# sauloal/pykmer

Measured on AMD Instinct MI355X. Metric: bp/s k-mer counted (k=15, 1 GPU), higher is better.
Workload: dtype u8

## Files before the change

pykmer_amd/csrc/kmer_part.hip:

```cpp
#include <cstddef>
#include "part_common.h"

namespace pk {

__global__ __launch_bounds__(1024) void k_sample2(const uint32_t *__restrict__ in, const uint32_t *__restrict__ bucket_base,
                                                  const uint32_t *__restrict__ bucket_end, PartPlan pl, uint32_t stride2,
                                                  uint32_t *__restrict__ tally, uint32_t *__restrict__ sampled_n,
                                                  const uint32_t *__restrict__ flags) {
    __shared__ uint32_t h[512];
    __shared__ uint32_t n_seen;
    if (flags[0]) return;
    const uint32_t b = blockIdx.x, lo = bucket_base[b], hi = bucket_end[b];
    if (threadIdx.x < 512) h[threadIdx.x] = 0;
    if (threadIdx.x == 0) n_seen = 0;
    __syncthreads();
    const uint32_t n_grp = (hi - lo + 255u) / 256u, n_sgrp = (n_grp + stride2 - 1u) / stride2;
    const uint32_t mask = pl.B2 - 1u, shift = pl.fb_bits, w = threadIdx.x >> 6, lane = threadIdx.x & 63u;
    uint32_t mine = 0;
    for (uint32_t s0 = 0; s0 < n_sgrp; s0 += 8u * 16u) {
        uint4 v[8];
        uint32_t n_ok[8];
#pragma unroll
        for (int u = 0; u < 8; u++) {
            const uint32_t sg = s0 + (uint32_t)u * 16u + w;
            const uint64_t i = (uint64_t)lo + (uint64_t)sg * stride2 * 256u + lane * 4u;
            n_ok[u] = (sg < n_sgrp && i < hi) ? (uint32_t)min((uint64_t)4, (uint64_t)hi - i) : 0u;
            v[u] = n_ok[u] ? *reinterpret_cast<const uint4 *>(in + i) : make_uint4(0, 0, 0, 0);
        }
#pragma unroll
        for (int u = 0; u < 8; u++) {
            const uint32_t r4[4] = {v[u].x, v[u].y, v[u].z, v[u].w};
#pragma unroll
            for (uint32_t e = 0; e < 4; e++)
                if (e < n_ok[u]) { atomicAdd(&h[(r4[e] >> shift) & mask], 1u); mine++; }
        }
    }
    for (int d = 32; d; d >>= 1) mine += __shfl_down(mine, d, 64);
    if ((threadIdx.x & 63) == 0 && mine) atomicAdd(&n_seen, mine);
    __syncthreads();
    if (threadIdx.x < pl.B2) tally[(uint64_t)b * pl.B2 + threadIdx.x] = h[threadIdx.x];
    if (threadIdx.x == 0) sampled_n[b] = n_seen;
}
__global__ __launch_bounds__(1024) void k_rooms2(const uint32_t *__restrict__ tally, const uint32_t *__restrict__ sampled_n,
                                                 const uint32_t *__restrict__ bucket_base, const uint32_t *__restrict__ bucket_end, PartPlan pl,
                                                 uint32_t stride2, uint32_t n_final, uint32_t *__restrict__ final_start,
                                                 uint32_t *__restrict__ cap2_end, uint32_t *__restrict__ block_tot, const uint32_t *__restrict__ flags) {
    __shared__ uint32_t wsum[16];
    if (flags[0]) return;
    const uint32_t i = blockIdx.x * 1024u + threadIdx.x;
    uint32_t room = 0;
    if (i < n_final) {
        const uint32_t b = i >> pl.b2, hcount = tally[i];
        if (stride2 == 1u) room = hcount;
        else {
            const uint32_t seen = sampled_n[b], n_b = bucket_end[b] - bucket_base[b];
            const unsigned long long est = seen ? (unsigned long long)((double)hcount * ((double)n_b / (double)seen)) + 1ull : 0ull;
            room = (uint32_t)(est + est / 4 + 4096u);
        }
        room = (room + 7u) & ~7u;
    }
    uint32_t inc = room;
    const int lane = threadIdx.x & 63, w = threadIdx.x >> 6;
#pragma unroll
    for (int d = 1; d < 64; d <<= 1) { const uint32_t o = __shfl_up(inc, d, 64); if (lane >= d) inc += o; }
    if (lane == 63) wsum[w] = inc;
    __syncthreads();
    uint32_t pre = 0, total = 0;
    for (int j = 0; j < 16; j++) { if (j < w) pre += wsum[j]; total += wsum[j]; }
    if (i < n_final) { final_start[i] = pre + inc - room; cap2_end[i] = room; }
    if (threadIdx.x == 0) block_tot[blockIdx.x] = total;
}
__global__ __launch_bounds__(1024) void k_bases2(uint32_t n_blocks, uint32_t n_final, PartPlan pl, uint32_t *__restrict__ block_tot,
                                                 uint32_t *__restrict__ final_start, uint32_t *__restrict__ flags) {
    __shared__ uint32_t wsum[16];
    if (flags[0]) return;
    const uint32_t v = threadIdx.x < n_blocks ? block_tot[threadIdx.x] : 0u;
    uint32_t inc = v;
    const int lane = threadIdx.x & 63, w = threadIdx.x >> 6;
#pragma unroll
    for (int d = 1; d < 64; d <<= 1) { const uint32_t o = __shfl_up(inc, d, 64); if (lane >= d) inc += o; }
    if (lane == 63) wsum[w] = inc;
    __syncthreads();
    uint32_t pre = 0, total = 0;
    for (int j = 0; j < 16; j++) { if (j < w) pre += wsum[j]; total += wsum[j]; }
    if (threadIdx.x < n_blocks) block_tot[threadIdx.x] = pre + inc - v;
    __shared__ unsigned long long total64;
    if (threadIdx.x == 0) total64 = 0ull;
    __syncthreads();
    unsigned long long mine = v;
    for (int d = 32; d; d >>= 1) mine += __shfl_down(mine, d, 64);
    if (lane == 0 && mine) atomicAdd(&total64, mine);
    __syncthreads();
    if (threadIdx.x == 0) {
        final_start[n_final] = total;
        if (total64 > pl.capacity2) flags[0] = 1u;
    }
}
__global__ __launch_bounds__(1024) void k_starts2(uint32_t n_final, const uint32_t *__restrict__ block_base, uint32_t *__restrict__ final_start,
                                                  uint32_t *__restrict__ cursor2, uint32_t *__restrict__ cap2_end, const uint32_t *__restrict__ flags) {
    if (flags[0]) return;
    const uint32_t i = blockIdx.x * 1024u + threadIdx.x;
    if (i >= n_final) return;
    const uint32_t a = block_base[blockIdx.x] + final_start[i];
    final_start[i] = a; cursor2[i] = a; cap2_end[i] = a + cap2_end[i];
}

template <int NT, int PER, bool REC24 = false>
__global__ __launch_bounds__(NT, 4) void k_scatter2(const uint32_t *__restrict__ in, const uint32_t *__restrict__ wg2_start,
                                                   const uint32_t *__restrict__ bucket_base, const uint32_t *__restrict__ bucket_end, PartPlan pl,
                                                   void *__restrict__ out, uint32_t *__restrict__ cursor, const uint32_t *__restrict__ cap_end,
                                                   uint32_t dump, uint32_t *__restrict__ flags) {
    extern __shared__ __attribute__((aligned(16))) uint8_t smem[];
    ScatterLds &L = *reinterpret_cast<ScatterLds *>(smem);
    if (flags[0]) return;
    const uint32_t B = pl.B2, shift = pl.fb_bits;
    const uint32_t low_mask = (1u << shift) - 1u;
    for (uint32_t i = threadIdx.x; i < 512; i += NT) { L.hist[i] = 0; L.run[i] = 0; }
    __syncthreads();
    typedef uint32_t Quad __attribute__((ext_vector_type(4)));
    typedef uint32_t Pair __attribute__((ext_vector_type(2)));
    const uint16_t *in_lo = reinterpret_cast<const uint16_t *>(in);
    const uint8_t *in_hi = reinterpret_cast<const uint8_t *>(in) + level1_hi_plane_offset(pl.capacity1);
    auto item = [&](uint32_t b, uint32_t lo, uint32_t hi) {
        auto fetch = [&](uint32_t win, Quad (&v)[PER / 4]) {
            const uint32_t v_hi = min(hi, win + (uint32_t)TILE);
#pragma unroll
            for (int j = 0; j < PER / 4; j++) {
                const uint32_t i = win + (threadIdx.x + j * NT) * 4u;
                v[j] = Quad{0u, 0u, 0u, 0u};
                if (i < v_hi) {
                    if (REC24) {
                        const Pair l = *reinterpret_cast<const Pair *>(in_lo + i);
                        v[j] = Quad{l.x, l.y, *reinterpret_cast<const uint32_t *>(in_hi + i), 0u};
                    } else v[j] = *reinterpret_cast<const Quad *>(in + i);
                }
            }
        };
        Quad nxt[PER / 4];
        auto settle = [&]() {
            __builtin_amdgcn_s_waitcnt(0x0F70);
#pragma unroll
            for (int j = 0; j < PER / 4; j++) asm volatile("" : "+v"(nxt[j]));
        };
        fetch(lo & ~3u, nxt);
        settle();
        for (uint32_t win = lo & ~3u; win < hi; win += TILE) {
            const uint32_t v_lo = max(lo, win), v_hi = min(hi, win + (uint32_t)TILE);
            const uint32_t n_tile = v_hi - v_lo;
            uint32_t r[PER];
#pragma unroll
            for (int j = 0; j < PER / 4; j++) {
                if (REC24) {
                    r[j * 4] = __builtin_amdgcn_perm(nxt[j].z, nxt[j].x, 0x0c040100u);
                    r[j * 4 + 1] = __builtin_amdgcn_perm(nxt[j].z, nxt[j].x, 0x0c050302u);
                    r[j * 4 + 2] = __builtin_amdgcn_perm(nxt[j].z, nxt[j].y, 0x0c060100u);
                    r[j * 4 + 3] = __builtin_amdgcn_perm(nxt[j].z, nxt[j].y, 0x0c070302u);
                } else { r[j * 4] = nxt[j].x; r[j * 4 + 1] = nxt[j].y; r[j * 4 + 2] = nxt[j].z; r[j * 4 + 3] = nxt[j].w; }
            }
            const bool full = v_lo == win && n_tile == (uint32_t)TILE;
            uint32_t okm = 0;
            if (!full) {
#pragma unroll
                for (int j = 0; j < PER / 4; j++) {
                    const uint32_t i = win + (threadIdx.x + j * NT) * 4u;
#pragma unroll
                    for (int e = 0; e < 4; e++) okm |= (i + e >= v_lo && i + e < v_hi) ? (1u << (j * 4 + e)) : 0u;
                }
            }
            if (win + TILE < hi) fetch(win + TILE, nxt);
            uint32_t *cl = cursor + (uint64_t)b * B;
            const uint32_t *ce = cap_end + (uint64_t)b * B;
            if (full) scatter_tile<uint32_t, false, NT, PER, 512, true, 8, REC24>(L, r, 0u, n_tile, shift, B, low_mask, true, out, settle, cl, ce, dump, flags);
            else scatter_tile<uint32_t, false, NT, PER, 512, false, 8, REC24>(L, r, okm, n_tile, shift, B, low_mask, true, out, settle, cl, ce, dump, flags);
        }
    };
    const uint32_t *pos = wg2_start;
    const uint32_t per = pl.B1 >> 3;
    const uint32_t o_lo = (blockIdx.x & 7u) * per, o_hi = o_lo + per, first = blockIdx.x >> 3, step = gridDim.x >> 3;
    const uint32_t w_end = pos[o_hi];
    for (uint32_t w = pos[o_lo] + first; w < w_end; w += step) {
        uint32_t a = o_lo, z = o_hi;
        while (z - a > 1) { const uint32_t m = (a + z) >> 1; if (pos[m] <= w) a = m; else z = m; }
        const uint32_t b = (a % per) * 8u + a / per;
        const uint64_t s = (uint64_t)bucket_base[b] + (uint64_t)(w - pos[a]) * pl.R2;
        const uint64_t e = min(s + pl.R2, (uint64_t)bucket_end[b]);
        item(b, (uint32_t)s, (uint32_t)e);
    }
}

constexpr uint32_t K6_PIECE = 65024;
constexpr int K6_BYTES_LDS = 65536 + 1024 + 128;

__device__ __forceinline__ int wave_sum_i32(int v) {
    v += __builtin_amdgcn_update_dpp(0, v, 0x128, 0xf, 0xf, false);
    v += __builtin_amdgcn_update_dpp(0, v, 0x124, 0xf, 0xf, false);
    v += __builtin_amdgcn_update_dpp(0, v, 0x122, 0xf, 0xf, false);
    v += __builtin_amdgcn_update_dpp(0, v, 0x121, 0xf, 0xf, false);
    return __builtin_amdgcn_readlane(v, 0) + __builtin_amdgcn_readlane(v, 16) + __builtin_amdgcn_readlane(v, 32) +
           __builtin_amdgcn_readlane(v, 48);
}

typedef unsigned short U16x2 __attribute__((ext_vector_type(2)));
__device__ __forceinline__ uint32_t clamp255_pair(uint32_t x) {
    const U16x2 lim = {255, 255};
    return __builtin_bit_cast(uint32_t, __builtin_elementwise_min(__builtin_bit_cast(U16x2, x), lim));
}
__device__ __forceinline__ uint32_t pack_low_bytes(uint32_t x0, uint32_t x1) {
    return __builtin_amdgcn_perm(x1, x0, 0x06040200u);
}

struct SliceTally {
    int d1 = 0, d2 = 0;
    __device__ __forceinline__ void add_dword(int *dh, uint32_t x, int sign) {
        uint32_t p0 = x & 0x01010101u, p1 = (x >> 1) & 0x01010101u;
        uint32_t rest = p0 & p1;
        const uint32_t high = x & 0xfcfcfcfcu;
        if (high) {
            const uint32_t big = (((high & 0x7f7f7f7fu) + 0x7f7f7f7fu) | high) & 0x80808080u;
            const uint32_t keep = ~(big >> 7);
            p0 &= keep; p1 &= keep;
            rest = (p0 & p1) | (big >> 7);
        }
        const int n1 = (int)__builtin_popcount(p0 & ~p1), n2 = (int)__builtin_popcount(p1 & ~p0);
        d1 += sign * n1; d2 += sign * n2;
        while (rest) {
            const int bit = __ffs(rest) - 1;
            atomicAdd(&dh[(x >> bit) & 0xffu], sign);
            rest &= rest - 1u;
        }
    }
};

template <int T, bool LEAN, bool NOREC = false>
__device__ __forceinline__ void bucket_count_body(const uint16_t *__restrict__ recs, const uint32_t *__restrict__ final_start,
                                                  const uint32_t *__restrict__ final_end, uint32_t fb_bits, uint32_t split_bits,
                                                  uint8_t *__restrict__ table8, uint32_t fresh, unsigned long long *__restrict__ hist_rep, uint8_t *smem,
                                                  int *dh, uint32_t wg) {
    uint32_t *cnt = reinterpret_cast<uint32_t *>(smem);
    const uint32_t fb = wg >> split_bits, part = wg & ((1u << split_bits) - 1u);
    const uint32_t start = final_start[fb], end = final_end ? final_end[fb] : final_start[fb + 1];
    const uint32_t part_bits = fb_bits - split_bits;
    const uint32_t n_addr = 1u << part_bits;
    uint8_t *slice = table8 + ((uint64_t)fb << fb_bits) + (uint64_t)part * n_addr;
    if (start == end) {
        if (fresh) {
            if (n_addr >= 16) for (uint32_t g = threadIdx.x; g < n_addr / 16; g += T) reinterpret_cast<uint4 *>(slice)[g] = make_uint4(0, 0, 0, 0);
            else for (uint32_t a = threadIdx.x; a < n_addr; a += T) slice[a] = 0;
        }
        return;
    }
    const uint32_t base = start & ~7u;
    const uint32_t i_first = base + threadIdx.x * 8;
    uint4 v_first = make_uint4(0, 0, 0, 0);
    if (i_first < min(base + K6_PIECE, end)) v_first = *reinterpret_cast<const uint4 *>(recs + i_first);
    const bool by_rec = NOREC ? false : (((end - start) >> split_bits) < n_addr / 4 || n_addr < 16);
    SliceTally tally;
    for (uint32_t i = threadIdx.x; i < 256; i += T) dh[i] = 0;
    if (fresh) {
        if (n_addr >= 8) for (uint32_t g = threadIdx.x; g < n_addr / 8; g += T) reinterpret_cast<uint4 *>(cnt)[g] = make_uint4(0, 0, 0, 0);
        else for (uint32_t a = threadIdx.x; a < max(n_addr / 2, 1u); a += T) cnt[a] = 0u;
    } else if (n_addr >= 16) {
        if (!by_rec) __syncthreads();
        for (uint32_t g = threadIdx.x; g < n_addr / 16; g += T) {
            uint4 v = reinterpret_cast<const uint4 *>(slice)[g];
            uint32_t w[4] = {v.x, v.y, v.z, v.w};
            if (!by_rec) {
#pragma unroll
                for (int q = 0; q < 4; q++) tally.add_dword(dh, w[q], -1);
            }
#pragma unroll
            for (int q = 0; q < 8; q++)
                cnt[g * 8 + q] = __builtin_amdgcn_perm(0u, w[q >> 1], (q & 1) ? 0x0c030c02u : 0x0c010c00u);
        }
    } else {
        for (uint32_t a = threadIdx.x; a < n_addr / 2; a += T) cnt[a] = slice[2 * a] | ((uint32_t)slice[2 * a + 1] << 16);
    }
    __syncthreads();
    auto bump = [&](uint32_t a, uint32_t n) {
        const uint32_t sh = 16u * (a & 1u);
        if (!by_rec) { atomicAdd(&cnt[a >> 1], n << sh); return; }
        int &d1 = tally.d1, &d2 = tally.d2;
        const uint32_t c = (atomicAdd(&cnt[a >> 1], n << sh) >> sh) & 0xffffu;
        const uint32_t oc = c > 255u ? 255u : c, nc = c + n > 255u ? 255u : c + n;
        if (oc == nc) return;
        if (nc == 1u) d1++;
        else if (nc == 2u && oc == 1u) { d2++; d1--; }
        else {
            atomicAdd(&dh[nc], 1);
            if (oc) atomicAdd(&dh[oc], -1);
        }
    };
    auto count8 = [&](const uint4 &v, uint32_t i) {
        const uint32_t w[4] = {v.x, v.y, v.z, v.w};
        if (LEAN && !by_rec) {
            const bool interior = i >= start && i + 8u <= end;
            uint8_t *cb = reinterpret_cast<uint8_t *>(cnt);
#pragma unroll
            for (int q = 0; q < 8; q++) {
                const uint32_t x = w[q >> 1];
                const uint32_t off = (q & 1) ? ((x >> 15) & 0x1fffcu) : ((x << 1) & 0x1fffcu);
                const uint32_t low = (q & 1) ? ((x >> 16) & 1u) : (x & 1u);
                uint32_t val = low * 0xffffu + 1u;
                if (!interior) val = (i + q >= start && i + q < end) ? val : 0u;
                __hip_atomic_fetch_add(reinterpret_cast<uint32_t *>(cb + off), val, __ATOMIC_RELAXED, __HIP_MEMORY_SCOPE_WORKGROUP);
            }
            return;
        }
        uint32_t pa = 0, pn = 0;
#pragma unroll
        for (int q = 0; q < 8; q++) {
            const uint32_t idx = i + q;
            const uint32_t full = (w[q >> 1] >> (16 * (q & 1))) & 0xffffu;
            const bool in = idx >= start && idx < end && (full >> part_bits) == part;
            const uint32_t a = full & (n_addr - 1u);
            if (in && pn && a == pa) pn++;
            else {
                if (pn) bump(pa, pn);
                pa = a; pn = in ? 1u : 0u;
            }
        }
        if (pn) bump(pa, pn);
    };
    auto count8_sparse = [&](const uint4 &v, uint32_t i) {
        const uint32_t w[4] = {v.x, v.y, v.z, v.w};
        uint32_t old[8];
        bool in[8];
// ... 163 lines not shown
        return;
    }
    for (uint32_t g = threadIdx.x; g < N_ADDR / 16; g += T) slice[g] = img[g];
    d1 = wave_sum_i32(d1); d2 = wave_sum_i32(d2);
    if ((threadIdx.x & 63) == 0) {
        if (d1) atomicAdd(&dh[1], d1);
        if (d2) atomicAdd(&dh[2], d2);
    }
    __syncthreads();
    for (uint32_t i = threadIdx.x; i < 256; i += T) {
        const int x = dh[i];
        if (x) atomicAdd(&hist_rep[(uint64_t)(blockIdx.x % HIST_REPLICAS) * 256 + i], (unsigned long long)(long long)x);
    }
}

__device__ __forceinline__ void hist_reduce(unsigned long long *__restrict__ hist_rep, unsigned long long *__restrict__ hist) {
    if (threadIdx.x >= 256) return;
    unsigned long long acc = 0;
    for (uint32_t r = 0; r < HIST_REPLICAS; r++) {
        acc += hist_rep[(uint64_t)r * 256 + threadIdx.x];
        hist_rep[(uint64_t)r * 256 + threadIdx.x] = 0ull;
    }
    if (acc) atomicAdd(&hist[threadIdx.x], acc);
}

constexpr uint32_t AS_SLOTS = 4096, AS_WGS = 64;

__device__ __forceinline__ void table_sat_add(uint8_t *table8, uint64_t addr, uint32_t cnt, int *dh) {
    unsigned int *word = reinterpret_cast<unsigned int *>(table8 + (addr & ~3ull));
    const uint32_t sh = (uint32_t)(addr & 3ull) * 8u;
    unsigned int old = *word;
    while (true) {
        uint32_t b = (old >> sh) & 0xffu;
        uint32_t nb = b + cnt > 255u ? 255u : b + cnt;
        if (nb == b) return;
        unsigned int want = (old & ~(0xffu << sh)) | (nb << sh);
        unsigned int prev = atomicCAS(word, old, want);
        if (prev == old) {
            atomicAdd(&dh[nb], 1);
            if (b) atomicAdd(&dh[b], -1);
            return;
        }
        old = prev;
    }
}

__global__ __launch_bounds__(WG) void k_apply_side(const unsigned long long *__restrict__ side, const unsigned long long *__restrict__ side_n,
                                                   uint64_t side_cap, uint8_t *__restrict__ table8, unsigned long long *__restrict__ hist,
                                                   unsigned long long *__restrict__ hist_rep, const uint32_t *__restrict__ flags) {
    __shared__ unsigned long long key[AS_SLOTS];
    if (flags[0]) return;
    static_assert(WG >= 256, "one thread per histogram bin");
    if (blockIdx.x == 0) hist_reduce(hist_rep, hist);
    __shared__ uint32_t val[AS_SLOTS];
    __shared__ int dh[256];
    unsigned long long n = *side_n;
    if (n > side_cap) n = side_cap;
    const unsigned long long per = (n + gridDim.x - 1) / gridDim.x;
    const unsigned long long lo = per * blockIdx.x, hi = lo + per < n ? lo + per : n;
    if (lo >= hi) return;
    for (uint32_t i = threadIdx.x; i < AS_SLOTS; i += WG) { key[i] = 0ull; val[i] = 0u; }
    dh[threadIdx.x & 255u] = 0;
    __syncthreads();
    for (unsigned long long i = lo + threadIdx.x; i < hi; i += WG) {
        const unsigned long long e = side[i];
        const uint64_t addr = e >> SIDE_CNT_BITS;
        const uint32_t cnt = (uint32_t)(e & ((1ull << SIDE_CNT_BITS) - 1ull));
        const unsigned long long kk = addr + 1ull;
        uint32_t h = (uint32_t)((addr * 0x9E3779B97F4A7C15ull) >> 40) & (AS_SLOTS - 1u);
        bool done = false;
        for (uint32_t t = 0; t < 32 && !done; t++) {
            unsigned long long old = atomicCAS(&key[h], 0ull, kk);
            if (old == 0ull || old == kk) {
                uint32_t before = atomicAdd(&val[h], cnt);
                if (before + cnt < before) atomicExch(&val[h], 0xffffffffu);
                done = true;
            }
            h = (h + 1u) & (AS_SLOTS - 1u);
        }
        if (!done) table_sat_add(table8, addr, cnt > 255u ? 255u : cnt, dh);
    }
    __syncthreads();
    for (uint32_t i = threadIdx.x; i < AS_SLOTS; i += WG)
        if (key[i] != 0ull) table_sat_add(table8, key[i] - 1ull, val[i] > 255u ? 255u : val[i], dh);
    __syncthreads();
    if (threadIdx.x < 256 && dh[threadIdx.x]) atomicAdd(&hist[threadIdx.x], (unsigned long long)(long long)dh[threadIdx.x]);
}

PartPlan make_part_plan(uint32_t k, uint64_t n_bytes, uint32_t slice_bits, uint32_t slice_index) {
    PartPlan pl;
    pl.k = k;
    pl.slice_bits = slice_bits;
    pl.slice_index = slice_index;
    pl.addr_bits = 2 * k - slice_bits;
    pl.fb_bits = pl.addr_bits < 16 ? pl.addr_bits : 16;
    if (k <= 15 && pl.addr_bits >= 24 && n_bytes >= (((uint64_t)1 << pl.addr_bits) >> 3)) pl.fb_bits = 15;
    const uint32_t bucket_bits = pl.addr_bits - pl.fb_bits;
    const uint32_t one_level_max = k <= 15 ? 7u : 9u;
    pl.b1 = bucket_bits <= one_level_max ? bucket_bits : (bucket_bits + 1) / 2;
    if (pl.b1 > one_level_max) pl.b1 = one_level_max;
    pl.b2 = bucket_bits - pl.b1;
    pl.B1 = 1u << pl.b1;
    pl.B2 = 1u << pl.b2;
    pl.n_chunks = (uint32_t)((n_bytes + CHUNK - 1) / CHUNK);
    pl.n_wg0 = pl.n_chunks < 1024u ? pl.n_chunks : 1024u;
    if (pl.n_wg0 == 0) pl.n_wg0 = 1;
    pl.G = (pl.n_chunks + pl.n_wg0 - 1) / pl.n_wg0;
    if (pl.G == 0) pl.G = 1;
    const uint32_t wg1 = 4096u;
    pl.n_wg1 = pl.n_chunks < wg1 ? pl.n_chunks : wg1;
    if (pl.n_wg1 == 0) pl.n_wg1 = 1;
    pl.G1 = (pl.n_chunks + pl.n_wg1 - 1) / pl.n_wg1;
    if (pl.G1 == 0) pl.G1 = 1;
    pl.R2 = 4u * TILE;
    pl.sample_stride = pl.n_chunks >= 1024u ? 16u : 1u;
    const uint64_t nfb = (uint64_t)pl.B1 * pl.B2;
    pl.n_tally = (pl.b2 && nfb <= 32768 && pl.addr_bits <= 30) ? (uint32_t)nfb : pl.B1;
    pl.sample2 = (pl.b2 && pl.n_tally == pl.B1 && nfb <= 262144 && pl.B1 >= 8u) ? 1u : 0u;
    const uint64_t est1 = (uint64_t)pl.n_chunks * TILE + pl.B1, est2 = (uint64_t)pl.n_chunks * TILE + nfb;
    pl.capacity1 = est1 + est1 / 8 + (uint64_t)pl.B1 * 4100;
    pl.capacity2 = pl.sample2 ? est2 + est2 / 4 + nfb * 4104 : est2 + est2 / 8 + nfb * 2056;
    return pl;
}

size_t part_workspace_bytes(const PartPlan &pl, uint64_t n_bytes, PartWorkspace *lay) {
    auto up = [](size_t x) { return (x + 255) & ~(size_t)255; };
    const uint64_t nfb = (uint64_t)pl.B1 * pl.B2;
    size_t o = 0;
    lay->codes = o; o += up((size_t)pl.n_chunks * SLOT_CODE_WORDS * 4);
    lay->restarts = o; o += up((size_t)pl.n_chunks * SLOT_RST_WORDS * 4);
    lay->n_bases = o; o += up((size_t)pl.n_chunks * 4);
    lay->tally_rows = o; o += up((size_t)COUNT_WGS * pl.n_tally * 4);
    lay->tally_tot = o; o += up(pl.sample2 ? (size_t)nfb * 4 + (size_t)(pl.B1 + 1024) * 4 : (size_t)pl.n_tally * 4);
    lay->bucket_base = o; o += up((size_t)(pl.B1 + 1) * 4);
    lay->bucket_end = o; o += up((size_t)(pl.B1 + 1) * 4);
    lay->cursor1 = o; o += up((size_t)(pl.B1 + 1) * 4);
    lay->cap_end = o; o += up((size_t)(pl.B1 + 1) * 4);
    lay->wg2_start = o; o += up((size_t)(pl.B1 + 1) * 4);
    lay->final_start = o; o += up((size_t)(nfb + 1) * 4);
    lay->cursor2 = o; o += up((size_t)(nfb + 1) * 4);
    lay->cap2_end = o; o += up((size_t)(nfb + 1) * 4);
    lay->out1 = o; o += !pl.b2 ? up((size_t)(pl.capacity1 + TILE + 64) * 2)
                     : pl.k <= 15 ? level1_hi_plane_offset(pl.capacity1) + up((size_t)(pl.capacity1 + TILE + 64))
                                  : up((size_t)(pl.capacity1 + TILE + 64) * 4);
    lay->out2 = o; o += up(!pl.b2 ? 256 : (size_t)(pl.capacity2 + TILE + 64) * 2);
    lay->side_cap = n_bytes + 16;
    lay->side = o; o += up((size_t)lay->side_cap * 8);
    lay->side_n = o; o += 256;
    return o;
}

void part_set_attributes() {
    fuse_set_attributes();
    hipFuncSetAttribute((const void *)k_scatter2<512, 32>, hipFuncAttributeMaxDynamicSharedMemorySize, (int)SCATTER_LDS_NARROW);
    hipFuncSetAttribute((const void *)k_scatter2<512, 32, true>, hipFuncAttributeMaxDynamicSharedMemorySize, (int)SCATTER_LDS_NARROW);
    hipFuncSetAttribute((const void *)k_bucket_count<1024>, hipFuncAttributeMaxDynamicSharedMemorySize, 128 * 1024);
    hipFuncSetAttribute((const void *)k_bucket_count_half_lean<1024, true>, hipFuncAttributeMaxDynamicSharedMemorySize, 128 * 1024);
    hipFuncSetAttribute((const void *)k_bucket_count_half_lean<1024, false>, hipFuncAttributeMaxDynamicSharedMemorySize, 128 * 1024);
    hipFuncSetAttribute((const void *)k_bucket_count_bytes<1024>, hipFuncAttributeMaxDynamicSharedMemorySize, K6_BYTES_LDS);
}

extern "C" int pk_diag_occupancy(int which) {
    int n = -1;
    hipError_t e = hipErrorInvalidValue;
    if (which == 0) e = hipOccupancyMaxActiveBlocksPerMultiprocessor(&n, (const void *)k_bucket_count<1024>, 1024, 128 * 1024);
    if (which == 1) e = hipOccupancyMaxActiveBlocksPerMultiprocessor(&n, (const void *)k_bucket_count_bytes<1024>, 1024, K6_BYTES_LDS);
    if (which == 2) e = hipOccupancyMaxActiveBlocksPerMultiprocessor(&n, (const void *)k_bucket_count_half_lean<1024, true>, 1024, 65536);
    if (which == 3) e = hipOccupancyMaxActiveBlocksPerMultiprocessor(&n, (const void *)k_scatter2<512, 32>, 512, SCATTER_LDS_NARROW);
    return e == hipSuccess ? n : -(int)e;
}

int launch_partitioned(const L2 *st2, uint64_t n_bytes, const PartPlan &pl, uint32_t stride, uint8_t *ws, const PartWorkspace &lay, uint8_t *table8,
                       hipStream_t s, hipEvent_t ev_sort_begin, hipEvent_t ev_sort_end, hipEvent_t ev_part_end, bool fresh,
                       unsigned long long *hist, unsigned long long *bucket_hist, bool armed) {
    const uint32_t *codes = (const uint32_t *)(ws + lay.codes), *restarts = (const uint32_t *)(ws + lay.restarts);
    const uint32_t *n_bases = (const uint32_t *)(ws + lay.n_bases);
    uint32_t *tally_rows = (uint32_t *)(ws + lay.tally_rows), *tally_tot = (uint32_t *)(ws + lay.tally_tot);
    uint32_t *bucket_base = (uint32_t *)(ws + lay.bucket_base), *bucket_end = (uint32_t *)(ws + lay.bucket_end);
    uint32_t *cursor1 = (uint32_t *)(ws + lay.cursor1), *cap_end = (uint32_t *)(ws + lay.cap_end);
    uint32_t *wg2_start = (uint32_t *)(ws + lay.wg2_start), *final_start = (uint32_t *)(ws + lay.final_start);
    uint32_t *cursor2 = (uint32_t *)(ws + lay.cursor2), *cap2_end = (uint32_t *)(ws + lay.cap2_end);
    void *out1 = ws + lay.out1, *out2 = ws + lay.out2;
    unsigned long long *side = (unsigned long long *)(ws + lay.side), *side_n = (unsigned long long *)(ws + lay.side_n);
    uint32_t *flags = (uint32_t *)(side_n + 1);
    const uint32_t nfb = pl.B1 * pl.B2;
    const bool laid_out2 = pl.n_tally > pl.B1 || pl.sample2;
    if (pl.B1 > (pl.k <= 15 ? 128u : 512u) || pl.B2 > 512u || pl.fb_bits > 16u) return -3;
    if (pl.b2 && !laid_out2) return -3;
    if (pl.k <= 15 && pl.b2 && pl.addr_bits - pl.b1 > 24u) return -3;
    if (!armed && hipMemsetAsync(side_n, 0, PART_FLAG_WORDS * 4, s) != hipSuccess) return -2;
    launch_provision(codes, restarts, n_bases, st2, pl, stride, tally_rows, tally_tot, bucket_base, cursor1, cap_end, final_start, cursor2, cap2_end,
                     flags, s);
    if (ev_sort_begin) hipEventRecord(ev_sort_begin, s);
    launch_walk_sort(codes, restarts, n_bases, st2, pl, out1, cursor1, cap_end, flags, bucket_base, bucket_end, wg2_start, side, side_n, lay.side_cap, s);
    if (ev_sort_end) hipEventRecord(ev_sort_end, s);
    const uint16_t *final_recs = (const uint16_t *)out1;
    const uint32_t *k6_start = bucket_base, *k6_end = bucket_end;
    if (pl.sample2) {
        const uint32_t stride2 = stride == 1u ? 1u : 16u, n_blocks = (nfb + 1023u) / 1024u;
        uint32_t *sampled_n = tally_tot + nfb, *block_tot = sampled_n + pl.B1;
        hipLaunchKernelGGL(k_sample2, dim3(pl.B1), dim3(1024), 0, s, (const uint32_t *)out1, (const uint32_t *)bucket_base, (const uint32_t *)bucket_end,
                           pl, stride2, tally_tot, sampled_n, (const uint32_t *)flags);
        hipLaunchKernelGGL(k_rooms2, dim3(n_blocks), dim3(1024), 0, s, (const uint32_t *)tally_tot, (const uint32_t *)sampled_n,
                           (const uint32_t *)bucket_base, (const uint32_t *)bucket_end, pl, stride2, nfb, final_start, cap2_end, block_tot,
                           (const uint32_t *)flags);
        hipLaunchKernelGGL(k_bases2, dim3(1), dim3(1024), 0, s, n_blocks, nfb, pl, block_tot, final_start, flags);
        hipLaunchKernelGGL(k_starts2, dim3(n_blocks), dim3(1024), 0, s, nfb, (const uint32_t *)block_tot, final_start, cursor2, cap2_end,
                           (const uint32_t *)flags);
    }
    if (pl.b2) {
        const uint32_t grid2 = 4096u;
        if (pl.k <= 15)
            hipLaunchKernelGGL((k_scatter2<512, 32, true>), dim3(grid2), dim3(512), SCATTER_LDS_NARROW, s, (const uint32_t *)out1, wg2_start,
                               bucket_base, bucket_end, pl, out2, cursor2, (const uint32_t *)cap2_end, (uint32_t)pl.capacity2, flags);
        else
            hipLaunchKernelGGL((k_scatter2<512, 32>), dim3(grid2), dim3(512), SCATTER_LDS_NARROW, s, (const uint32_t *)out1, wg2_start,
                               bucket_base, bucket_end, pl, out2, cursor2, (const uint32_t *)cap2_end, (uint32_t)pl.capacity2, flags);
        final_recs = (const uint16_t *)out2; k6_start = final_start; k6_end = cursor2;
    }
    if (ev_part_end) hipEventRecord(ev_part_end, s);
    const bool sparse = pl.fb_bits == 16 && n_bytes / nfb < 8192u;
    const uint32_t split = sparse ? 1u : 0u;
    const size_t part_addrs = (size_t)1 << (pl.fb_bits - split);
    const size_t lds6 = part_addrs * 2 < 64 ? 64 : part_addrs * 2;
    const uint32_t n_rows6 = (uint32_t)(nfb << split);
    if (split > 1u) return -3;
    if (pl.fb_bits == 15 && fresh)
        hipLaunchKernelGGL((k_bucket_count_half_lean<1024, true>), dim3(n_rows6), dim3(1024), lds6, s, final_recs, k6_start, k6_end, pl.fb_bits, split, table8,
                           fresh ? 1u : 0u, bucket_hist, (const uint32_t *)flags);
    else if (pl.fb_bits == 15)
        hipLaunchKernelGGL((k_bucket_count_half_lean<1024, false>), dim3(n_rows6), dim3(1024), lds6, s, final_recs, k6_start, k6_end, pl.fb_bits, split, table8,
                           fresh ? 1u : 0u, bucket_hist, (const uint32_t *)flags);
    else if (split)
        hipLaunchKernelGGL(k_bucket_count_bytes<1024>, dim3(nfb), dim3(1024), K6_BYTES_LDS, s, final_recs, k6_start, k6_end, table8, fresh ? 1u : 0u, bucket_hist,
                           (const uint32_t *)flags);
    else
        hipLaunchKernelGGL(k_bucket_count<1024>, dim3(n_rows6), dim3(1024), lds6, s, final_recs, k6_start, k6_end, pl.fb_bits, split, table8,
                           fresh ? 1u : 0u, bucket_hist, (const uint32_t *)flags);
    hipLaunchKernelGGL(k_apply_side, dim3(AS_WGS), dim3(WG), 0, s, side, side_n, lay.side_cap, table8, hist, bucket_hist, (const uint32_t *)flags);
    return hipGetLastError() == hipSuccess ? 0 : -2;
}

}
```

pykmer_amd/csrc/part_common.h:

```cpp
#pragma once
#include <cstddef>
#include "fasta_fsm.h"
#include "pk_kernels.h"

namespace pk {

constexpr int SC_T = 1024;
constexpr int SC_PER = 16;
constexpr int TILE = SC_T * SC_PER;

constexpr uint32_t HOT_PROBES = 16;
constexpr uint32_t SIDE_CNT_BITS = 28;

template <uint32_t SLOTS>
struct HotTable {
    static constexpr uint32_t HOT_SLOTS = SLOTS;
    unsigned long long key[SLOTS];
    uint32_t val[SLOTS];
    uint32_t used, n_flush;
    unsigned long long flush_base;
};

__device__ __forceinline__ void side_append_one(unsigned long long *side, unsigned long long *side_n, uint64_t side_cap,
                                                uint64_t addr, uint32_t cnt) {
    unsigned long long i = atomicAdd(side_n, 1ull);
    if (i < side_cap) side[i] = ((unsigned long long)addr << SIDE_CNT_BITS) | cnt;
}

template <uint32_t SLOTS>
__device__ __forceinline__ void hot_insert(HotTable<SLOTS> &H, uint64_t addr, uint32_t cnt, unsigned long long *side,
                                           unsigned long long *side_n, uint64_t side_cap) {
    constexpr uint32_t HOT_SLOTS = SLOTS;
    const unsigned long long key = addr + 1ull;
    uint32_t h = (uint32_t)((addr * 0x9E3779B97F4A7C15ull) >> 40) & (HOT_SLOTS - 1u);
#pragma unroll 1
    for (uint32_t t = 0; t < HOT_PROBES; t++) {
        unsigned long long old = atomicCAS(&H.key[h], 0ull, key);
        if (old == 0ull || old == key) {
            if (old == 0ull) atomicAdd(&H.used, 1u);
            atomicAdd(&H.val[h], cnt);
            return;
        }
        h = (h + 1u) & (HOT_SLOTS - 1u);
    }
    side_append_one(side, side_n, side_cap, addr, cnt);
}

template <uint32_t SLOTS>
__device__ __forceinline__ void hot_flush(HotTable<SLOTS> &H, unsigned long long *side, unsigned long long *side_n, uint64_t side_cap) {
    constexpr uint32_t HOT_SLOTS = SLOTS;
    __syncthreads();
    if (threadIdx.x == 0) H.n_flush = 0;
    __syncthreads();
    uint32_t mine = 0;
    for (uint32_t i = threadIdx.x; i < HOT_SLOTS; i += blockDim.x) mine += H.key[i] != 0ull;
    uint32_t at = mine ? atomicAdd(&H.n_flush, mine) : 0u;
    __syncthreads();
    if (threadIdx.x == 0) H.flush_base = H.n_flush ? atomicAdd(side_n, (unsigned long long)H.n_flush) : 0ull;
    __syncthreads();
    const unsigned long long base64 = H.flush_base;
    for (uint32_t i = threadIdx.x; i < HOT_SLOTS; i += blockDim.x) {
        if (H.key[i] != 0ull) {
            unsigned long long dst = base64 + at++;
            if (dst < side_cap) side[dst] = ((H.key[i] - 1ull) << SIDE_CNT_BITS) | H.val[i];
            H.key[i] = 0ull; H.val[i] = 0u;
        }
    }
    if (threadIdx.x == 0) H.used = 0;
    __syncthreads();
}


__host__ __device__ __forceinline__ size_t level1_hi_plane_offset(uint64_t capacity1) {
    return (((size_t)(capacity1 + TILE + 64) * 2u) + 255u) & ~(size_t)255u;
}

__device__ __forceinline__ uint32_t wave_incl_scan_u32(uint32_t v) {
    v += (uint32_t)__builtin_amdgcn_update_dpp(0, (int)v, 0x111, 0xf, 0xf, false);
    v += (uint32_t)__builtin_amdgcn_update_dpp(0, (int)v, 0x112, 0xf, 0xf, false);
    v += (uint32_t)__builtin_amdgcn_update_dpp(0, (int)v, 0x114, 0xf, 0xf, false);
    v += (uint32_t)__builtin_amdgcn_update_dpp(0, (int)v, 0x118, 0xf, 0xf, false);
    v += (uint32_t)__builtin_amdgcn_update_dpp(0, (int)v, 0x142, 0xa, 0xf, false);
    v += (uint32_t)__builtin_amdgcn_update_dpp(0, (int)v, 0x143, 0xc, 0xf, false);
    return v;
}

template <int NB>
struct ScatterLdsT {
    uint32_t hist[NB + 64], off[NB + 64], run[NB], gbase[NB];
    uint32_t wsum[SC_T / 64];
    uint32_t total, pad_[3];
    uint32_t rec[TILE + 64];
    uint16_t dig[TILE + 64];
};
typedef ScatterLdsT<512> ScatterLds;
constexpr size_t SCATTER_LDS_NARROW = offsetof(ScatterLds, dig);
constexpr size_t SCATTER_LDS_WIDE = sizeof(ScatterLds);

template <typename RIN, bool WIDE, int NT = SC_T, int PER = SC_PER, int NB = 512, bool FULL = false, int SB = 0, bool OFF32 = false, class Settle>
__device__ __forceinline__ void scatter_tile(ScatterLdsT<NB> &L, const RIN (&r)[PER], uint32_t okm, uint32_t n_tile,
                                             uint32_t shift, uint32_t B, uint32_t low_mask, bool out16, void *__restrict__ out,
                                             Settle &&settle, uint32_t *claim = nullptr, const uint32_t *__restrict__ cap_end = nullptr,
                                             uint32_t dump = 0, uint32_t *overflow = nullptr, uint8_t *__restrict__ out_hi = nullptr,
                                             const uint32_t *watch = nullptr, uint32_t watch_limit = 0,
                                             bool *watch_hit = nullptr) {
    static_assert(NT * PER == TILE, "tile shape");
    const uint32_t lane = threadIdx.x & 63u;
    const uint32_t dbits = (uint32_t)__builtin_ctz(B);
    auto digit_of = [&](const RIN &x) -> uint32_t {
        return sizeof(RIN) == 4 ? __builtin_amdgcn_ubfe((uint32_t)x, shift, dbits) : (uint32_t)((uint64_t)x >> shift) & (B - 1u);
    };
    constexpr bool BRANCH_FREE = PER <= 16;
    constexpr bool KEEP_DG = PER <= 16 && sizeof(RIN) == 4;
    uint32_t dg[KEEP_DG ? PER : 1];
    auto slot_digit = [&](int j) -> uint32_t { return (FULL || ((okm >> j) & 1u)) ? digit_of(r[j]) : (uint32_t)NB + lane; };
    if (BRANCH_FREE) {
        if (KEEP_DG) {
#pragma unroll
            for (int j = 0; j < PER; j++) dg[KEEP_DG ? j : 0] = slot_digit(j);
        }
#pragma unroll
        for (int j = 0; j < PER; j++)
            __hip_atomic_fetch_add(&L.hist[KEEP_DG ? dg[KEEP_DG ? j : 0] : slot_digit(j)], 1u, __ATOMIC_RELAXED, __HIP_MEMORY_SCOPE_WORKGROUP);
    } else {
#pragma unroll
        for (int j = 0; j < PER; j++)
            if (FULL || ((okm >> j) & 1u)) __hip_atomic_fetch_add(&L.hist[digit_of(r[j])], 1u, __ATOMIC_RELAXED, __HIP_MEMORY_SCOPE_WORKGROUP);
    }
    if (!FULL && threadIdx.x < 64u) L.off[NB + threadIdx.x] = (uint32_t)TILE + threadIdx.x;
    __syncthreads();
    if (watch && threadIdx.x == 0) L.pad_[0] = *watch >= watch_limit ? 1u : 0u;
    uint32_t my_off = 0, claimed = 0, room_end = 0, run_len = 0;
    {
        uint32_t tid = threadIdx.x;
        asm volatile("" : "+v"(tid));
        const int lane = tid & 63, w = tid >> 6;
        const uint32_t v = threadIdx.x < B ? L.hist[threadIdx.x] : 0u;
        const uint32_t inc = wave_incl_scan_u32(v);
        if (lane == 63) L.wsum[w] = inc;
        __syncthreads();
        uint32_t pre = 0;
        for (int i = 0; i < w; i++) pre += L.wsum[i];
        my_off = pre + inc - v;
        if (threadIdx.x < B) {
            L.off[threadIdx.x] = my_off;
            if (threadIdx.x == B - 1u) L.total = my_off + v;
            if (claim) {
                claimed = v ? atomicAdd(reinterpret_cast<uint32_t *>(reinterpret_cast<uint8_t *>(claim) + tid * 4u), v) : 0u;
                if (cap_end) room_end = *reinterpret_cast<const uint32_t *>(reinterpret_cast<const uint8_t *>(cap_end) + tid * 4u);
                run_len = v;
            } else { L.gbase[threadIdx.x] = L.run[threadIdx.x] - my_off; L.run[threadIdx.x] += v; }
            L.hist[threadIdx.x] = 0;
        }
    }
    __syncthreads();
    if (watch_hit) *watch_hit = L.pad_[0] != 0u;
    if (n_tile == ~0u) n_tile = L.total;
    n_tile = (uint32_t)__builtin_amdgcn_readfirstlane((int)n_tile);
    if (BRANCH_FREE) {
#pragma unroll
        for (int j = 0; j < PER; j++) {
            const uint32_t d = KEEP_DG ? dg[KEEP_DG ? j : 0] : slot_digit(j);
            const uint32_t p = atomicAdd(&L.off[d], (FULL || ((okm >> j) & 1u)) ? 1u : 0u);
            if (WIDE) { L.rec[p] = (uint32_t)((uint64_t)r[j] & low_mask); L.dig[p] = (uint16_t)d; }
            else L.rec[p] = (uint32_t)r[j];
        }
    } else {
#pragma unroll
        for (int j = 0; j < PER; j++)
            if (FULL || ((okm >> j) & 1u)) {
                const uint32_t d = digit_of(r[j]);
                const uint32_t p = atomicAdd(&L.off[d], 1u);
                if (WIDE) { L.rec[p] = (uint32_t)((uint64_t)r[j] & low_mask); L.dig[p] = (uint16_t)d; }
                else L.rec[p] = (uint32_t)r[j];
            }
    }
    if (claim && threadIdx.x < B) {
        if (cap_end && run_len && claimed + run_len > room_end) {
            *overflow = 1u;
            claimed = dump + my_off;
        }
        L.gbase[threadIdx.x] = claimed - my_off;
    }
    __syncthreads();
    settle();
    auto store_runs = [&](auto *o) {
        constexpr bool O16 = sizeof(*o) == 2;
        const bool planes = O16 && !out16;
        auto put = [&](uint32_t at, uint32_t v) {
            if (OFF32) *reinterpret_cast<decltype(o)>(reinterpret_cast<uint8_t *>(o) + (uint32_t)(at * (uint32_t)sizeof(*o))) = (decltype(*o + 0))v;
            else o[at] = v;
        };
        auto idx32 = [](uint32_t at) -> uint32_t { return at; };
        if constexpr (SB == 0) {
#pragma unroll
            for (int j = 0; j < PER; j++) {
                const uint32_t p = threadIdx.x + (uint32_t)j * NT;
                if (p < n_tile) {
                    const uint32_t r0 = L.rec[p];
                    const uint32_t d0 = WIDE ? (uint32_t)L.dig[p] : __builtin_amdgcn_ubfe(r0, shift, dbits);
                    const uint32_t at = idx32(p + L.gbase[d0]);
                    if (O16) { put(at, (uint16_t)(planes ? r0 : (r0 & low_mask))); if (planes) out_hi[at] = (uint8_t)(r0 >> 16); }
                    else put(at, r0);
                }
            }
        } else {
            static_assert(SB == 0 || PER % (SB ? SB : 1) == 0, "store batch");
#pragma unroll
            for (int j0 = 0; j0 < PER; j0 += (SB ? SB : 1)) {
                uint32_t r0[SB ? SB : 1], g0[SB ? SB : 1];
#pragma unroll
                for (int u = 0; u < SB; u++) r0[u] = L.rec[threadIdx.x + (uint32_t)(j0 + u) * NT];
#pragma unroll
                for (int u = 0; u < SB; u++) {
                    const uint32_t p = threadIdx.x + (uint32_t)(j0 + u) * NT;
                    const uint32_t d0 = WIDE ? ((uint32_t)L.dig[p] & (uint32_t)(NB - 1)) : __builtin_amdgcn_ubfe(r0[u], shift, dbits);
                    g0[u] = L.gbase[d0];
                }
                const bool whole = !FULL && (uint32_t)(j0 + SB) * NT <= n_tile;
                if (whole) {
#pragma unroll
                    for (int u = 0; u < SB; u++) {
                        const uint32_t p = threadIdx.x + (uint32_t)(j0 + u) * NT;
                        const uint32_t at = idx32(p + g0[u]);
                        if (O16) { put(at, (uint16_t)(planes ? r0[u] : (r0[u] & low_mask))); if (planes) out_hi[at] = (uint8_t)(r0[u] >> 16); }
                        else put(at, r0[u]);
                    }
                } else {
#pragma unroll
                    for (int u = 0; u < SB; u++) {
                        const uint32_t p = threadIdx.x + (uint32_t)(j0 + u) * NT;
                        if (FULL || p < n_tile) {
                            const uint32_t at = idx32(p + g0[u]);
                            if (O16) { put(at, (uint16_t)(planes ? r0[u] : (r0[u] & low_mask))); if (planes) out_hi[at] = (uint8_t)(r0[u] >> 16); }
                            else put(at, r0[u]);
                        }
                    }
                }
            }
        }
    };
    if (out16 || out_hi) store_runs(reinterpret_cast<uint16_t *>(out));
    else store_runs(reinterpret_cast<uint32_t *>(out));
}


}
```

Before: 216.8 billion.

## Use per-lane-column private LDS counters in level-2 scatter to cut atomic contention

Replaces the single shared histogram and offset array in the level-2 scatter with C replicated counters per digit, indexed by thread column (8 copies for the 24-bit k<=15 path with 256 digits, 4 copies otherwise). This spreads LDS atomics across banks and copies, reducing same-address contention when many threads hit the same digit. The scan now reads quad vectors of counters, computes per-copy exclusive offsets in place, and reduces across lanes to get per-digit totals for the global claim. The cost is a larger histogram region that must be zeroed after every tile, one extra barrier, and B2 capped at 256 for k<=15.

```diff
diff --git a/pykmer_amd/csrc/kmer_part.hip b/pykmer_amd/csrc/kmer_part.hip
--- a/pykmer_amd/csrc/kmer_part.hip
+++ b/pykmer_amd/csrc/kmer_part.hip
@@ -1,4 +1,5 @@
 #include <cstddef>
+#include <type_traits>
 #include "part_common.h"
 
 namespace pk {
@@ -111,11 +112,13 @@
                                                    void *__restrict__ out, uint32_t *__restrict__ cursor, const uint32_t *__restrict__ cap_end,
                                                    uint32_t dump, uint32_t *__restrict__ flags) {
     extern __shared__ __attribute__((aligned(16))) uint8_t smem[];
-    ScatterLds &L = *reinterpret_cast<ScatterLds *>(smem);
+    typedef std::conditional_t<REC24, Scatter2Lds24, Scatter2Lds> Lds;
+    constexpr int NB = REC24 ? 256 : 512, C = REC24 ? 8 : 4;
+    Lds &L = *reinterpret_cast<Lds *>(smem);
     if (flags[0]) return;
     const uint32_t B = pl.B2, shift = pl.fb_bits;
     const uint32_t low_mask = (1u << shift) - 1u;
-    for (uint32_t i = threadIdx.x; i < 512; i += NT) { L.hist[i] = 0; L.run[i] = 0; }
+    for (uint32_t i = threadIdx.x; i < NB * C; i += NT) L.hist[i] = 0;
     __syncthreads();
     typedef uint32_t Quad __attribute__((ext_vector_type(4)));
     typedef uint32_t Pair __attribute__((ext_vector_type(2)));
@@ -170,8 +173,8 @@
             if (win + TILE < hi) fetch(win + TILE, nxt);
             uint32_t *cl = cursor + (uint64_t)b * B;
             const uint32_t *ce = cap_end + (uint64_t)b * B;
-            if (full) scatter_tile<uint32_t, false, NT, PER, 512, true, 8, REC24>(L, r, 0u, n_tile, shift, B, low_mask, true, out, settle, cl, ce, dump, flags);
-            else scatter_tile<uint32_t, false, NT, PER, 512, false, 8, REC24>(L, r, okm, n_tile, shift, B, low_mask, true, out, settle, cl, ce, dump, flags);
+            if (full) scatter_tile<uint32_t, false, NT, PER, NB, true, 8, REC24, C>(L, r, 0u, n_tile, shift, B, low_mask, true, out, settle, cl, ce, dump, flags);
+            else scatter_tile<uint32_t, false, NT, PER, NB, false, 8, REC24, C>(L, r, okm, n_tile, shift, B, low_mask, true, out, settle, cl, ce, dump, flags);
         }
     };
     const uint32_t *pos = wg2_start;
@@ -641,8 +644,8 @@
 
 void part_set_attributes() {
     fuse_set_attributes();
-    hipFuncSetAttribute((const void *)k_scatter2<512, 32>, hipFuncAttributeMaxDynamicSharedMemorySize, (int)SCATTER_LDS_NARROW);
-    hipFuncSetAttribute((const void *)k_scatter2<512, 32, true>, hipFuncAttributeMaxDynamicSharedMemorySize, (int)SCATTER_LDS_NARROW);
+    hipFuncSetAttribute((const void *)k_scatter2<512, 32>, hipFuncAttributeMaxDynamicSharedMemorySize, (int)SCATTER2_LDS);
+    hipFuncSetAttribute((const void *)k_scatter2<512, 32, true>, hipFuncAttributeMaxDynamicSharedMemorySize, (int)SCATTER2_LDS_24);
     hipFuncSetAttribute((const void *)k_bucket_count<1024>, hipFuncAttributeMaxDynamicSharedMemorySize, 128 * 1024);
     hipFuncSetAttribute((const void *)k_bucket_count_half_lean<1024, true>, hipFuncAttributeMaxDynamicSharedMemorySize, 128 * 1024);
     hipFuncSetAttribute((const void *)k_bucket_count_half_lean<1024, false>, hipFuncAttributeMaxDynamicSharedMemorySize, 128 * 1024);
@@ -655,7 +658,8 @@
     if (which == 0) e = hipOccupancyMaxActiveBlocksPerMultiprocessor(&n, (const void *)k_bucket_count<1024>, 1024, 128 * 1024);
     if (which == 1) e = hipOccupancyMaxActiveBlocksPerMultiprocessor(&n, (const void *)k_bucket_count_bytes<1024>, 1024, K6_BYTES_LDS);
     if (which == 2) e = hipOccupancyMaxActiveBlocksPerMultiprocessor(&n, (const void *)k_bucket_count_half_lean<1024, true>, 1024, 65536);
-    if (which == 3) e = hipOccupancyMaxActiveBlocksPerMultiprocessor(&n, (const void *)k_scatter2<512, 32>, 512, SCATTER_LDS_NARROW);
+    if (which == 3) e = hipOccupancyMaxActiveBlocksPerMultiprocessor(&n, (const void *)k_scatter2<512, 32, true>, 512, SCATTER2_LDS_24);
+    if (which == 4) e = hipOccupancyMaxActiveBlocksPerMultiprocessor(&n, (const void *)k_scatter2<512, 32>, 512, SCATTER2_LDS);
     return e == hipSuccess ? n : -(int)e;
 }
 
@@ -674,7 +678,7 @@
     uint32_t *flags = (uint32_t *)(side_n + 1);
     const uint32_t nfb = pl.B1 * pl.B2;
     const bool laid_out2 = pl.n_tally > pl.B1 || pl.sample2;
-    if (pl.B1 > (pl.k <= 15 ? 128u : 512u) || pl.B2 > 512u || pl.fb_bits > 16u) return -3;
+    if (pl.B1 > (pl.k <= 15 ? 128u : 512u) || pl.B2 > (pl.k <= 15 ? 256u : 512u) || pl.fb_bits > 16u) return -3;
     if (pl.b2 && !laid_out2) return -3;
     if (pl.k <= 15 && pl.b2 && pl.addr_bits - pl.b1 > 24u) return -3;
     if (!armed && hipMemsetAsync(side_n, 0, PART_FLAG_WORDS * 4, s) != hipSuccess) return -2;
@@ -700,10 +704,10 @@
     if (pl.b2) {
         const uint32_t grid2 = 4096u;
         if (pl.k <= 15)
-            hipLaunchKernelGGL((k_scatter2<512, 32, true>), dim3(grid2), dim3(512), SCATTER_LDS_NARROW, s, (const uint32_t *)out1, wg2_start,
+            hipLaunchKernelGGL((k_scatter2<512, 32, true>), dim3(grid2), dim3(512), SCATTER2_LDS_24, s, (const uint32_t *)out1, wg2_start,
                                bucket_base, bucket_end, pl, out2, cursor2, (const uint32_t *)cap2_end, (uint32_t)pl.capacity2, flags);
         else
-            hipLaunchKernelGGL((k_scatter2<512, 32>), dim3(grid2), dim3(512), SCATTER_LDS_NARROW, s, (const uint32_t *)out1, wg2_start,
+            hipLaunchKernelGGL((k_scatter2<512, 32>), dim3(grid2), dim3(512), SCATTER2_LDS, s, (const uint32_t *)out1, wg2_start,
                                bucket_base, bucket_end, pl, out2, cursor2, (const uint32_t *)cap2_end, (uint32_t)pl.capacity2, flags);
         final_recs = (const uint16_t *)out2; k6_start = final_start; k6_end = cursor2;
     }
diff --git a/pykmer_amd/csrc/part_common.h b/pykmer_amd/csrc/part_common.h
--- a/pykmer_amd/csrc/part_common.h
+++ b/pykmer_amd/csrc/part_common.h
@@ -85,20 +85,24 @@
     return v;
 }
 
-template <int NB>
+template <int NB, int C = 0>
 struct ScatterLdsT {
-    uint32_t hist[NB + 64], off[NB + 64], run[NB], gbase[NB];
+    uint32_t hist[C ? NB * C : NB + 64], off[C ? NB : NB + 64], run[C ? 4 : NB], gbase[NB];
     uint32_t wsum[SC_T / 64];
     uint32_t total, pad_[3];
     uint32_t rec[TILE + 64];
     uint16_t dig[TILE + 64];
 };
 typedef ScatterLdsT<512> ScatterLds;
-constexpr size_t SCATTER_LDS_NARROW = offsetof(ScatterLds, dig);
 constexpr size_t SCATTER_LDS_WIDE = sizeof(ScatterLds);
-
-template <typename RIN, bool WIDE, int NT = SC_T, int PER = SC_PER, int NB = 512, bool FULL = false, int SB = 0, bool OFF32 = false, class Settle>
-__device__ __forceinline__ void scatter_tile(ScatterLdsT<NB> &L, const RIN (&r)[PER], uint32_t okm, uint32_t n_tile,
+typedef ScatterLdsT<256, 8> Scatter2Lds24;
+typedef ScatterLdsT<512, 4> Scatter2Lds;
+constexpr size_t SCATTER2_LDS_24 = offsetof(Scatter2Lds24, dig);
+constexpr size_t SCATTER2_LDS = offsetof(Scatter2Lds, dig);
+
+template <typename RIN, bool WIDE, int NT = SC_T, int PER = SC_PER, int NB = 512, bool FULL = false, int SB = 0, bool OFF32 = false, int C = 0,
+          class Settle>
+__device__ __forceinline__ void scatter_tile(ScatterLdsT<NB, C> &L, const RIN (&r)[PER], uint32_t okm, uint32_t n_tile,
                                              uint32_t shift, uint32_t B, uint32_t low_mask, bool out16, void *__restrict__ out,
                                              Settle &&settle, uint32_t *claim = nullptr, const uint32_t *__restrict__ cap_end = nullptr,
                                              uint32_t dump = 0, uint32_t *overflow = nullptr, uint8_t *__restrict__ out_hi = nullptr,
@@ -112,6 +116,16 @@
     };
     constexpr bool BRANCH_FREE = PER <= 16;
     constexpr bool KEEP_DG = PER <= 16 && sizeof(RIN) == 4;
+    static_assert(C == 0 || (!BRANCH_FREE && !WIDE && NB * C == 4 * NT && (C & (C - 1)) == 0 && C <= 32), "bank-private counters");
+    auto col_base = [&]() -> uint32_t {
+        uint32_t t = threadIdx.x;
+        asm volatile("" : "+v"(t));
+        return (t & (uint32_t)(C ? C - 1 : 0)) * 4u;
+    };
+    auto ctr = [&](uint32_t d, uint32_t cbase) -> uint32_t * {
+        constexpr uint32_t CS = C ? (uint32_t)__builtin_ctz(C) + 2u : 2u;
+        return C ? reinterpret_cast<uint32_t *>(reinterpret_cast<uint8_t *>(L.hist) + ((d << CS) + cbase)) : &L.hist[d];
+    };
     uint32_t dg[KEEP_DG ? PER : 1];
     auto slot_digit = [&](int j) -> uint32_t { return (FULL || ((okm >> j) & 1u)) ? digit_of(r[j]) : (uint32_t)NB + lane; };
     if (BRANCH_FREE) {
@@ -123,11 +137,12 @@
         for (int j = 0; j < PER; j++)
             __hip_atomic_fetch_add(&L.hist[KEEP_DG ? dg[KEEP_DG ? j : 0] : slot_digit(j)], 1u, __ATOMIC_RELAXED, __HIP_MEMORY_SCOPE_WORKGROUP);
     } else {
+        const uint32_t cbase = C ? col_base() : 0u;
 #pragma unroll
         for (int j = 0; j < PER; j++)
-            if (FULL || ((okm >> j) & 1u)) __hip_atomic_fetch_add(&L.hist[digit_of(r[j])], 1u, __ATOMIC_RELAXED, __HIP_MEMORY_SCOPE_WORKGROUP);
-    }
-    if (!FULL && threadIdx.x < 64u) L.off[NB + threadIdx.x] = (uint32_t)TILE + threadIdx.x;
+            if (FULL || ((okm >> j) & 1u)) __hip_atomic_fetch_add(ctr(digit_of(r[j]), cbase), 1u, __ATOMIC_RELAXED, __HIP_MEMORY_SCOPE_WORKGROUP);
+    }
+    if (BRANCH_FREE && !FULL && threadIdx.x < 64u) L.off[NB + threadIdx.x] = (uint32_t)TILE + threadIdx.x;
     __syncthreads();
     if (watch && threadIdx.x == 0) L.pad_[0] = *watch >= watch_limit ? 1u : 0u;
     uint32_t my_off = 0, claimed = 0, room_end = 0, run_len = 0;
@@ -135,22 +150,48 @@
         uint32_t tid = threadIdx.x;
         asm volatile("" : "+v"(tid));
         const int lane = tid & 63, w = tid >> 6;
-        const uint32_t v = threadIdx.x < B ? L.hist[threadIdx.x] : 0u;
-        const uint32_t inc = wave_incl_scan_u32(v);
-        if (lane == 63) L.wsum[w] = inc;
-        __syncthreads();
-        uint32_t pre = 0;
-        for (int i = 0; i < w; i++) pre += L.wsum[i];
-        my_off = pre + inc - v;
-        if (threadIdx.x < B) {
-            L.off[threadIdx.x] = my_off;
-            if (threadIdx.x == B - 1u) L.total = my_off + v;
-            if (claim) {
-                claimed = v ? atomicAdd(reinterpret_cast<uint32_t *>(reinterpret_cast<uint8_t *>(claim) + tid * 4u), v) : 0u;
-                if (cap_end) room_end = *reinterpret_cast<const uint32_t *>(reinterpret_cast<const uint8_t *>(cap_end) + tid * 4u);
-                run_len = v;
-            } else { L.gbase[threadIdx.x] = L.run[threadIdx.x] - my_off; L.run[threadIdx.x] += v; }
-            L.hist[threadIdx.x] = 0;
+        if constexpr (C > 0) {
+            typedef uint32_t Quad __attribute__((ext_vector_type(4)));
+            constexpr uint32_t G = C / 4, GS = (uint32_t)__builtin_ctz(G);
+            Quad *q4 = reinterpret_cast<Quad *>(reinterpret_cast<uint8_t *>(L.hist) + tid * 16u);
+            const Quad c4 = *q4;
+            const uint32_t s = c4.x + c4.y + c4.z + c4.w;
+            const uint32_t inc = wave_incl_scan_u32(s);
+            if (lane == 63) L.wsum[w] = inc;
+            __syncthreads();
+            uint32_t pre = 0;
+            for (int i = 0; i < w; i++) pre += L.wsum[i];
+            const uint32_t ex = pre + inc - s;
+            *q4 = Quad{ex, ex + c4.x, ex + c4.x + c4.y, ex + c4.x + c4.y + c4.z};
+            uint32_t v = s;
+#pragma unroll
+            for (uint32_t m = 1; m < G; m <<= 1) v += (uint32_t)__shfl_xor((int)v, (int)m);
+            const uint32_t d = tid >> GS;
+            if ((tid & (G - 1u)) == 0u && d < B) {
+                L.gbase[d] = ex;
+                L.off[d] = v;
+                if (d == B - 1u) L.total = ex + v;
+                claimed = v ? atomicAdd(reinterpret_cast<uint32_t *>(reinterpret_cast<uint8_t *>(claim) + d * 4u), v) : 0u;
+                if (cap_end) room_end = *reinterpret_cast<const uint32_t *>(reinterpret_cast<const uint8_t *>(cap_end) + d * 4u);
+            }
+        } else {
+            const uint32_t v = threadIdx.x < B ? L.hist[threadIdx.x] : 0u;
+            const uint32_t inc = wave_incl_scan_u32(v);
+            if (lane == 63) L.wsum[w] = inc;
+            __syncthreads();
+            uint32_t pre = 0;
+            for (int i = 0; i < w; i++) pre += L.wsum[i];
+            my_off = pre + inc - v;
+            if (threadIdx.x < B) {
+                L.off[threadIdx.x] = my_off;
+                if (threadIdx.x == B - 1u) L.total = my_off + v;
+                if (claim) {
+                    claimed = v ? atomicAdd(reinterpret_cast<uint32_t *>(reinterpret_cast<uint8_t *>(claim) + tid * 4u), v) : 0u;
+                    if (cap_end) room_end = *reinterpret_cast<const uint32_t *>(reinterpret_cast<const uint8_t *>(cap_end) + tid * 4u);
+                    run_len = v;
+                } else { L.gbase[threadIdx.x] = L.run[threadIdx.x] - my_off; L.run[threadIdx.x] += v; }
+                L.hist[threadIdx.x] = 0;
+            }
         }
     }
     __syncthreads();
@@ -166,23 +207,36 @@
             else L.rec[p] = (uint32_t)r[j];
         }
     } else {
+        const uint32_t cbase = C ? col_base() : 0u;
 #pragma unroll
         for (int j = 0; j < PER; j++)
             if (FULL || ((okm >> j) & 1u)) {
                 const uint32_t d = digit_of(r[j]);
-                const uint32_t p = atomicAdd(&L.off[d], 1u);
+                const uint32_t p = atomicAdd(C ? ctr(d, cbase) : &L.off[d], 1u);
                 if (WIDE) { L.rec[p] = (uint32_t)((uint64_t)r[j] & low_mask); L.dig[p] = (uint16_t)d; }
                 else L.rec[p] = (uint32_t)r[j];
             }
     }
-    if (claim && threadIdx.x < B) {
+    constexpr uint32_t GS = C ? (uint32_t)__builtin_ctz(C / 4) : 0u;
+    uint32_t ct = threadIdx.x;
+    if (C) asm volatile("" : "+v"(ct));
+    const uint32_t cd = ct >> GS;
+    if (claim && cd < B && (ct & ((1u << GS) - 1u)) == 0u) {
+        if (C) { my_off = L.gbase[cd]; run_len = L.off[cd]; }
         if (cap_end && run_len && claimed + run_len > room_end) {
             *overflow = 1u;
             claimed = dump + my_off;
         }
-        L.gbase[threadIdx.x] = claimed - my_off;
-    }
-    __syncthreads();
+        L.gbase[cd] = claimed - my_off;
+    }
+    __syncthreads();
+    if constexpr (C > 0) {
+        typedef uint32_t Quad __attribute__((ext_vector_type(4)));
+        uint32_t t = threadIdx.x, z = 0u;
+        asm volatile("" : "+v"(t), "+v"(z));
+        *reinterpret_cast<Quad *>(reinterpret_cast<uint8_t *>(L.hist) + t * 16u) = Quad{z, z, z, z};
+        __syncthreads();
+    }
     settle();
     auto store_runs = [&](auto *o) {
         constexpr bool O16 = sizeof(*o) == 2;
```

After: 220.7 billion (median of 6 runs). 1.8% higher.
